# Video-Object-Detection/TSCD

Hardware: NVIDIA B200
Metric: clip-frames/sec of TSCD aggregation stage (higher is better)
Workload: dtype f16

## Files before the change

include/tscd_b200.h:

```cpp
#ifndef TSCD_B200_H_
#define TSCD_B200_H_

#include <stdint.h>

#ifdef __cplusplus
extern "C" {
#endif

#define TSCD_OK 0
#define TSCD_ERR_INVALID_ARG (-1)
#define TSCD_ERR_UNSUPPORTED (-2)
#define TSCD_ERR_CAPACITY (-3)
#define TSCD_ERR_CUDA (-4)

#define TSCD_F32 0
#define TSCD_F16 1
#define TSCD_BF16 2

#define TSCD_MAX_LEVELS 3

typedef struct {
    const void* ptr[TSCD_MAX_LEVELS];
    int64_t frame_stride[TSCD_MAX_LEVELS];
    int64_t anchor_stride[TSCD_MAX_LEVELS];
// ... 153 lines not shown
typedef struct {
    tscd_attn_layout lay;
    int32_t rows;
    const int32_t* m_dev;
    const void* x;
    int64_t ldx;
    const void* w;
    const int32_t* row_meta;
    const float* key_score;
    float scale;
    void *qn, *kn, *vn;
    void* vt;
    void* xori;
    int32_t ld_xori;
} tscd_qkv_project_args;
int tscd_qkv_project(const tscd_qkv_project_args* args, void* stream);

typedef struct {
    tscd_attn_layout lay;
    int32_t* row_frame;
    int32_t* row_meta;
    void* vt_cls;
    void* vt_reg;
} tscd_attn_rowmeta_args;
int tscd_attn_rowmeta(const tscd_attn_rowmeta_args* args, void* stream);

typedef struct {
    tscd_attn_layout lay;
    const void *qn_cls, *kn_cls, *qn_reg, *kn_reg;
    const void *vt_cls, *vt_reg;
    const int32_t* row_frame;
    int32_t need_reg;
    void* x_cls;
    void* x_reg;
    int32_t ld_x;
    float* stats;
    float max_logit;
} tscd_attn_pv_args;
int tscd_attn_pv(const tscd_attn_pv_args* args, void* stream);

typedef struct {
    tscd_attn_layout lay;
    const void *qn_cls, *kn_cls, *qn_reg, *kn_reg, *vn_cls, *vn_reg;
    const void* vt;
    const int32_t* row_frame;
    const float* stats;
    int32_t use_obj_mask;
    float sim_thresh;
    float conf_sim_thresh;
    void* out;
    int32_t ld_out;
    void* w_out;
    const void* w_in;
} tscd_attn_round2_args;
int tscd_attn_round2(const tscd_attn_round2_args* args, void* stream);

typedef struct {
    tscd_attn_layout lay;
    int32_t width;
    const void* x;
    int32_t ld_x;
    void* xt;
} tscd_transpose_args;
int tscd_transpose_clip(const tscd_transpose_args* args, void* stream);

typedef struct {
    int32_t B, F, L, D;
    int32_t bank_dtype;
    const int32_t* row_off;
    const int32_t* lrow_off;
    const void* bank_reg;
    const void* bank_edge;
    const float* time_emb;
    const float* se_w1;
    const float* se_w2;
    const float* emb_reg;
    const float* emb_cls;
    float* feat;
    float* edge;
    void* feat16;
    void* kin16;
    float* kin;
    float* norm_reg;
    float* norm_cls;
    int32_t emb_dtype;
} tscd_cafm_prep_args;
int tscd_cafm_prep(const tscd_cafm_prep_args* args, void* stream);

typedef struct {
    int32_t B, L, D, kmax;
    const int32_t* lrow_off;
    const int32_t* resume;
    const int32_t* st_n;
    const float* emb_reg; const float* emb_cls; const float* norm_reg; const float* norm_cls;
    const float* st_reg; const float* st_cls; const float* st_nreg; const float* st_ncls;
    float* cost;
    int32_t* ref_n;
    int32_t emb_dtype;
    const void* emb_reg16;
    const void* emb_cls16;
    int32_t emb16_dtype;
} tscd_cafm_cost_args;
int tscd_cafm_cost(const tscd_cafm_cost_args* args, void* stream);

typedef struct {
    int32_t num_frames, kmax;
// ... 246 lines not shown
```

tscd_b200/_lib.py:

```python
import ctypes as C
import os

from .build import LIB_PATH

TSCD_F32, TSCD_F16, TSCD_BF16 = 0, 1, 2
MAX_LEVELS = 3
_ERR = {-1: "invalid argument", -2: "unsupported configuration", -3: "capacity exceeded", -4: "CUDA error"}


class View(C.Structure):
    _fields_ = [("ptr", C.c_void_p * MAX_LEVELS), ("frame_stride", C.c_int64 * MAX_LEVELS),
                ("anchor_stride", C.c_int64 * MAX_LEVELS), ("chan_stride", C.c_int64 * MAX_LEVELS)]


class Anchors(C.Structure):
    _fields_ = [("num_levels", C.c_int32), ("level_h", C.c_int32 * MAX_LEVELS), ("level_w", C.c_int32 * MAX_LEVELS),
                ("level_stride", C.c_int32 * MAX_LEVELS), ("level_start", C.c_int32 * (MAX_LEVELS + 1))]


class SelectArgs(C.Structure):
    _fields_ = [("mode", C.c_int32), ("num_frames", C.c_int32), ("num_classes", C.c_int32), ("head_dtype", C.c_int32),
                ("apply_sigmoid", C.c_int32), ("apply_decode", C.c_int32), ("pre_k", C.c_int32),
                ("conf_thresh", C.c_float), ("minimal_limit", C.c_int32), ("maximal_limit", C.c_int32),
                ("cand_cap", C.c_int32), ("anchors", Anchors), ("reg", View), ("obj", View), ("cls", View),
# ... 23 lines not shown
                ("bank_dtype", C.c_int32), ("anchors", Anchors), ("reg", View), ("obj", View), ("cls", View),
                ("feat_cls", View), ("feat_reg", View), ("feat_edge", View),
                ("cand_idx", C.c_void_p), ("cand_count", C.c_void_p), ("keep", C.c_void_p), ("keep_count", C.c_void_p),
                ("sel_count", C.c_void_p), ("row_off", C.c_void_p), ("sel_idx", C.c_void_p), ("sel_rows", C.c_void_p),
                ("bank_cls", C.c_void_p), ("bank_reg", C.c_void_p), ("bank_edge", C.c_void_p),
                ("bank_score", C.c_void_p), ("bank_fg", C.c_void_p), ("bank_box", C.c_void_p)]


class LinearArgs(C.Structure):
    _fields_ = [("M", C.c_int32), ("N", C.c_int32), ("K", C.c_int32), ("dtype", C.c_int32),
                ("x", C.c_void_p), ("ldx", C.c_int64), ("w", C.c_void_p), ("ldw", C.c_int64),
                ("bias", C.c_void_p), ("m_dev", C.c_void_p), ("out16", C.c_void_p), ("ld16", C.c_int32),
                ("out32", C.c_void_p), ("ld32", C.c_int32)]


class AttnLayout(C.Structure):
    _fields_ = [("B", C.c_int32), ("F", C.c_int32), ("L", C.c_int32), ("self_attn", C.c_int32), ("dtype", C.c_int32),
                ("row_cap", C.c_int32), ("nk_pitch", C.c_int32), ("row_off", C.c_void_p), ("lrow_off", C.c_void_p)]


class AttnPrepArgs(C.Structure):
    _fields_ = [("lay", AttnLayout), ("scale", C.c_float), ("qkv_cls", C.c_void_p), ("qkv_reg", C.c_void_p),
                ("ld_qkv", C.c_int32), ("key_score", C.c_void_p),
                ("qn_cls", C.c_void_p), ("kn_cls", C.c_void_p), ("vn_cls", C.c_void_p),
                ("qn_reg", C.c_void_p), ("kn_reg", C.c_void_p), ("vn_reg", C.c_void_p),
                ("vt_cls", C.c_void_p), ("vt_reg", C.c_void_p), ("xori_cls", C.c_void_p), ("xori_reg", C.c_void_p),
                ("ld_xori", C.c_int32), ("row_frame", C.c_void_p)]


class QkvProjectArgs(C.Structure):
    _fields_ = [("lay", AttnLayout), ("rows", C.c_int32), ("m_dev", C.c_void_p), ("x", C.c_void_p), ("ldx", C.c_int64),
                ("w", C.c_void_p), ("row_meta", C.c_void_p), ("key_score", C.c_void_p), ("scale", C.c_float),
                ("qn", C.c_void_p), ("kn", C.c_void_p), ("vn", C.c_void_p), ("vt", C.c_void_p), ("xori", C.c_void_p),
                ("ld_xori", C.c_int32)]


class AttnRowmetaArgs(C.Structure):
    _fields_ = [("lay", AttnLayout), ("row_frame", C.c_void_p), ("row_meta", C.c_void_p), ("vt_cls", C.c_void_p),
                ("vt_reg", C.c_void_p)]


class AttnPvArgs(C.Structure):
    _fields_ = [("lay", AttnLayout), ("qn_cls", C.c_void_p), ("kn_cls", C.c_void_p), ("qn_reg", C.c_void_p),
                ("kn_reg", C.c_void_p), ("vt_cls", C.c_void_p), ("vt_reg", C.c_void_p), ("row_frame", C.c_void_p),
                ("need_reg", C.c_int32), ("x_cls", C.c_void_p), ("x_reg", C.c_void_p), ("ld_x", C.c_int32),
                ("stats", C.c_void_p), ("max_logit", C.c_float)]


class AttnRound2Args(C.Structure):
    _fields_ = [("lay", AttnLayout), ("qn_cls", C.c_void_p), ("kn_cls", C.c_void_p), ("qn_reg", C.c_void_p),
                ("kn_reg", C.c_void_p), ("vn_cls", C.c_void_p), ("vn_reg", C.c_void_p), ("vt", C.c_void_p),
                ("row_frame", C.c_void_p), ("stats", C.c_void_p), ("use_obj_mask", C.c_int32),
                ("sim_thresh", C.c_float), ("conf_sim_thresh", C.c_float), ("out", C.c_void_p), ("ld_out", C.c_int32),
                ("w_out", C.c_void_p), ("w_in", C.c_void_p)]


class TransposeArgs(C.Structure):
    _fields_ = [("lay", AttnLayout), ("width", C.c_int32), ("x", C.c_void_p), ("ld_x", C.c_int32), ("xt", C.c_void_p)]


def _fields(spec):
    m = {"i": C.c_int32, "f": C.c_float, "p": C.c_void_p}
    return [(x.split(":")[0], m[x.split(":")[1]]) for x in spec.split()]


class CafmPrepArgs(C.Structure):
    _fields_ = _fields("B:i F:i L:i D:i bank_dtype:i row_off:p lrow_off:p bank_reg:p bank_edge:p time_emb:p se_w1:p "
                       "se_w2:p emb_reg:p emb_cls:p feat:p edge:p feat16:p kin16:p kin:p norm_reg:p norm_cls:p emb_dtype:i")


class CafmChainArgs(C.Structure):
    _fields_ = _fields("B:i F:i L:i D:i kmax:i out_dtype:i row_off:p lrow_off:p resume:p feat:p edge:p kin:p kproj:p "
                       "vproj:p kproj16:p vproj16:p wq16:p bank_reg:p bank_edge:p time_emb:p emb_reg:p emb_cls:p norm_reg:p norm_cls:p wq_t:p se_w1:p se_w2:p ln_w:p "
                       "ln_b:p dec_w:p dec_b:p st_n:p st_out:p st_edge:p st_reg:p st_cls:p st_nreg:p st_ncls:p "
                       "st_time:p sc_qin:p sc_q:p sc_k:p ref_n:p lap_col:p lap_row:p out16:p out32:p perm:p status:p emb_dtype:i")


class CafmWideArgs(C.Structure):
    _fields_ = [("base", CafmChainArgs)] + _fields("qin16:p attn:p q_beg:p q_end:p kv_beg:p kv_end:p ctl:p perm_s:p prow_s:p ord_prev:p "
                                                   "n_prev:p last_l0:p")


class FrameFlashArgs(C.Structure):
    _fields_ = _fields("num_items:i heads:i head_dim:i dtype:i max_q:i q_beg:p q_end:p kv_beg:p kv_end:p q:p ldq:i k:p ldk:i v:p ldv:i "
                       "out:p ldo:i")


class EdgePatchesArgs(C.Structure):
    _fields_ = [("num_frames", C.c_int32), ("max_keep", C.c_int32), ("feat_dtype", C.c_int32), ("op_dtype", C.c_int32),
                ("anchors", Anchors), ("feat_reg", View), ("sel_idx", C.c_void_p), ("sel_count", C.c_void_p), ("row_off", C.c_void_p),
                ("seg_base", C.c_int32 * MAX_LEVELS), ("seg_cap", C.c_int32 * MAX_LEVELS), ("level_count", C.c_void_p),
                ("slot", C.c_void_p), ("patches", C.c_void_p), ("hf", C.c_void_p), ("status", C.c_void_p)]


class EdgeCombineArgs(C.Structure):
    _fields_ = _fields("rows_cap:i op_dtype:i total_rows:p slot:p content:p hf_out:p bank_edge:p")


class CafmCostArgs(C.Structure):
    _fields_ = _fields("B:i L:i D:i kmax:i lrow_off:p resume:p st_n:p emb_reg:p emb_cls:p norm_reg:p norm_cls:p "
                       "st_reg:p st_cls:p st_nreg:p st_ncls:p cost:p ref_n:p emb_dtype:i emb_reg16:p emb_cls16:p emb16_dtype:i")


class CafmLapArgs(C.Structure):
    _fields_ = _fields("num_frames:i kmax:i lrow_off:p ref_n:p cost:p lap_col:p lap_row:p")


# ... 149 lines not shown
```

tscd_b200/aggregate.py:

```python
from typing import Dict, Optional

import torch

import os

SINGLE_PASS_MAX_LOGIT = float(os.environ.get("TSCD_ATTN_MAX_LOGIT", "25.0"))

from . import ops

FUSED_QKV = True


class MCAWeights:

    def __init__(self, sd: Dict[str, torch.Tensor], prefix: str, dtype=torch.float16, device="cuda"):
        def w(name):
            return sd[prefix + name].detach().to(device=device, dtype=dtype).contiguous()

        def b(name):
            return sd[prefix + name].detach().to(device=device, dtype=torch.float32).contiguous()

        self.qkv_cls = torch.cat([w("mca.q_cls_local.weight"), w("mca.kv_cls.weight")], 0).contiguous()
        self.qkv_reg = torch.cat([w("mca.q_reg_local.weight"), w("mca.kv_reg.weight")], 0).contiguous()
        self.lin_w, self.lin_b = w("mca.linear.weight"), b("mca.linear.bias")
# ... 28 lines not shown
                                     xori_cls=tmp_c[:, 256:], xori_reg=tmp_r[:, 256:], tag=tag)
    else:
        qkv_c, _ = ops.linear(bank_cls, w.qkv_cls, m_dev=n_rows_dev)
        qkv_r, _ = ops.linear(bank_reg, w.qkv_reg, m_dev=n_rows_dev)
        bufs = ops.attn_prep(lay, qkv_c, qkv_r, bank_score, xori_cls=tmp_c[:, 256:], xori_reg=tmp_r[:, 256:])
    stats = torch.empty(lay.loc_cap, 16, dtype=torch.float32, device=dev)
    ops.attn_pv(lay, bufs, tmp_c[:, :256], tmp_r[:, :256], stats, need_reg=need_reg, tag=tag, max_logit=SINGLE_PASS_MAX_LOGIT)
    cat_c = torch.empty(lay.loc_cap, 768, dtype=dt, device=dev)
    ops.linear(tmp_c, w.lin_w, w.lin_b, m_dev=n_loc_dev, out16=cat_c[:, 256:], want16=False, tag=tag + ".mca_linear")
    w_keep = torch.empty(lay.loc_cap, lay.nk_pitch, dtype=dt, device=dev) if need_reg else None
    ops.attn_round2(lay, bufs, bufs["vt_cls"], stats, cat_c[:, :256], use_obj_mask=False, sim_thresh=sim_thresh,
                    conf_sim_thresh=conf_sim_thresh, w_out=w_keep, tag=tag + ".cls")
    trans_cls16, trans_cls32 = ops.linear(cat_c, w.out_w, w.out_b, m_dev=n_loc_dev, want16=cls_out[0], want32=cls_out[1],
                                          tag=tag + ".linear")
    trans_obj16 = trans_obj32 = None
    cat_r = None
    if need_reg:
        cat_r = torch.empty(lay.loc_cap, 768, dtype=dt, device=dev)
        ops.linear(tmp_r, w.linreg_w, w.linreg_b, m_dev=n_loc_dev, out16=cat_r[:, 256:], want16=False, tag=tag + ".mca_linear_reg")
        ops.attn_round2(lay, bufs, bufs["vt_reg"], stats, cat_r[:, :256], use_obj_mask=True, sim_thresh=sim_thresh,
                        conf_sim_thresh=conf_sim_thresh, w_in=w_keep, tag=tag + ".obj")
        trans_obj16, trans_obj32 = ops.linear(cat_r, w.obj_w, w.obj_b, m_dev=n_loc_dev, want16=obj_out[0], want32=obj_out[1],
                                              tag=tag + ".linear_obj")
    if debug is not None:
        debug.update(qkv_c=qkv_c, qkv_r=qkv_r, bufs=bufs, tmp_c=tmp_c, tmp_r=tmp_r, stats=stats, cat_c=cat_c, cat_r=cat_r)
    return (trans_cls16, trans_cls32), (trans_obj16, trans_obj32)


class MSAWeights:

    def __init__(self, sd: Dict[str, torch.Tensor], prefix: str, dtype=torch.float16, device="cuda"):
        w = lambda n: sd[prefix + n].detach().to(device=device, dtype=dtype).contiguous()
        b = lambda n: sd[prefix + n].detach().to(device=device, dtype=torch.float32).contiguous()
        self.qkv_cls, self.qkv_reg = w("msa.qkv_cls.weight"), w("msa.qkv_reg.weight")
        self.l1_w, self.l1_b = w("linear1.weight"), b("linear1.bias")
        self.l2_w, self.l2_b = w("linear2.weight"), b("linear2.bias")


def msa_forward(lay: ops.AttnLayoutT, w: MSAWeights, bank_cls, bank_reg, bank_score, n_rows_dev,
                sim_thresh=0.75, conf_sim_thresh=0.99):
    assert lay.self_attn and lay.L == lay.F
    dev, dt, cap = bank_cls.device, lay.dtype, lay.row_cap
    qkv_c, _ = ops.linear(bank_cls, w.qkv_cls, m_dev=n_rows_dev, tag="msa.qkv_cls")
    qkv_r, _ = ops.linear(bank_reg, w.qkv_reg, m_dev=n_rows_dev, tag="msa.qkv_reg")
    tmp_c = torch.empty(cap, 512, dtype=dt, device=dev)
    tmp_r = torch.empty(cap, 512, dtype=dt, device=dev)
    bufs = ops.attn_prep(lay, qkv_c, qkv_r, bank_score, xori_cls=tmp_c[:, 256:], xori_reg=tmp_r[:, 256:])
    stats = torch.empty(cap, 16, dtype=torch.float32, device=dev)
    ops.attn_pv(lay, bufs, tmp_c[:, :256], tmp_r[:, :256], stats, need_reg=False, tag="msa", max_logit=SINGLE_PASS_MAX_LOGIT)
    cat = torch.empty(cap, 1024, dtype=dt, device=dev)
    ops.linear(tmp_c, w.l1_w, w.l1_b, m_dev=n_rows_dev, out16=cat[:, 512:], want16=False, tag="msa.linear1")
    tct = torch.empty(lay.B * 512, lay.nk_pitch, dtype=dt, device=dev)
    ops.call("tscd_transpose_clip", ops.L.TransposeArgs, lay=lay.to_c(), width=512, x=cat[:, 512:], ld_x=cat.stride(0), xt=tct)
    for half in range(2):
        vt = tct.view(lay.B, 512, lay.nk_pitch)[:, half * 256:(half + 1) * 256]
        vt = vt.contiguous().view(lay.B * 256, lay.nk_pitch)
        ops.attn_round2(lay, bufs, vt, stats, cat[:, half * 256:(half + 1) * 256], use_obj_mask=False,
                        sim_thresh=sim_thresh, conf_sim_thresh=conf_sim_thresh, tag=f"msa.half{half}")
    return ops.linear(cat, w.l2_w, w.l2_b, m_dev=n_rows_dev, want16=True, want32=True, tag="msa.linear2")
```

tscd_b200/csrc/attn.cu:

```cuda
#include <cuda.h>

#include "common.cuh"
#include "tc.cuh"

namespace tscd {

int make_tmap_kmajor(CUtensorMap* m, const void* ptr, int is_bf16, int64_t rows, int64_t K, int64_t ld, int box_rows);

constexpr int kAttnThreads = 160;
constexpr float kLog2e = 1.4426950408889634f;

template <typename T>
__device__ __forceinline__ float2 ld2(const T* p);
template <> __device__ __forceinline__ float2 ld2<__half>(const __half* p) { return __half22float2(*reinterpret_cast<const __half2*>(p)); }
template <> __device__ __forceinline__ float2 ld2<__nv_bfloat16>(const __nv_bfloat16* p) {
    return __bfloat1622float2(*reinterpret_cast<const __nv_bfloat162*>(p));
}
template <typename T>
__device__ __forceinline__ void st2(T* p, float a, float b);
template <> __device__ __forceinline__ void st2<__half>(__half* p, float a, float b) { *reinterpret_cast<__half2*>(p) = __floats2half2_rn(a, b); }
template <> __device__ __forceinline__ void st2<__nv_bfloat16>(__nv_bfloat16* p, float a, float b) {
    *reinterpret_cast<__nv_bfloat162*>(p) = __floats2bfloat162_rn(a, b);
}

// ... 544 lines not shown
            softmax_bar_sync();
            lc = (bars.xch[0][row] + bars.xch[1][row]) + (bars.xch[2][row] + bars.xch[3][row]);
            softmax_bar_sync();
            bars.xch[quarter][row] = lr;
            softmax_bar_sync();
            lr = (bars.xch[0][row] + bars.xch[1][row]) + (bars.xch[2][row] + bars.xch[3][row]);
            softmax_bar_sync();
            lsum_c[h] = lc; lsum_r[h] = lr;
            PV_WAIT(&bars.o_full, h & 1, 352);
            tc_fence_after();
            const float ic = 0.5f / lc, ir = 0.5f / lr;
            for (int br = 0; br < (need_reg ? 2 : 1); ++br) {
                uint16_t* dst = reinterpret_cast<uint16_t*>(br == 0 ? a.x_cls : a.x_reg);
                const int c0 = quarter * 16;
                uint32_t oc[16], orr[16];
                tmem_ld_32x16(lane_base + (need_reg ? 256 + br * 64 : 256) + c0, oc);
                tmem_ld_32x16(lane_base + (need_reg ? 384 + br * 64 : 320) + c0, orr);
                tmem_ld_wait();
                if (q_ok) {
                    uint32_t pk[8];
#pragma unroll
                    for (int j = 0; j < 8; ++j)
                        pk[j] = pack2<BF16>(__uint_as_float(oc[2 * j]) * ic + __uint_as_float(orr[2 * j]) * ir,
                                            __uint_as_float(oc[2 * j + 1]) * ic + __uint_as_float(orr[2 * j + 1]) * ir);
                    uint4* o = reinterpret_cast<uint4*>(dst + (int64_t)(ci.lbase + q) * a.ld_x + h * 64 + c0);
#pragma unroll
                    for (int j = 0; j < 2; ++j) o[j] = make_uint4(pk[4 * j], pk[4 * j + 1], pk[4 * j + 2], pk[4 * j + 3]);
                }
            }
            tc_fence_before();
            __syncwarp();
            if (lane == 0) mbar_arrive(&bars.o_empty);
        }
        if (q_ok && quarter == 0) {
            float4* st = reinterpret_cast<float4*>(a.stats + (int64_t)(ci.lbase + q) * 16);
            st[0] = make_float4(mxc[0], mxc[1], mxc[2], mxc[3]);
            st[1] = make_float4(mxr[0], mxr[1], mxr[2], mxr[3]);
            st[2] = make_float4(lsum_c[0], lsum_c[1], lsum_c[2], lsum_c[3]);
            st[3] = make_float4(lsum_r[0], lsum_r[1], lsum_r[2], lsum_r[3]);
        }
    }
#ifdef TSCD_R2_PROF
    if (blockIdx.x == 0 && blockIdx.y == 0 && threadIdx.x == 0) atomicAdd(&g_pv_wait[63], (unsigned long long)(clock64() - tk0));
#endif
    tc_fence_before();
    __syncthreads();
    if (warp == 17) {
        tc_fence_after();
        tmem_dealloc<512>(tmem);
    }
}

struct R2Tmaps {
    CUtensorMap q128c, q128r, k64c, k64r, vn128c, vn128r, vn64c, vn64r, vt;
};

constexpr int kR2Threads = 640;
constexpr int kR2MaxSlots = 16;
constexpr int kR2SlotBytes = 8192;
constexpr int kR2SmemBytes = 229376;

struct R2Bars {
    uint64_t full[kR2MaxSlots], empty[kR2MaxSlots];
    uint64_t res_full;
    uint64_t r_full[2], r_empty[2];
    uint64_t s_full[2], s_empty[2];
    uint64_t w_full[2], w_empty[2];
    uint64_t u_full;
    uint32_t tmem_base;
    float xch[4][128];
};

static_assert(kR2SmemBytes + sizeof(R2Bars) <= 232448, "attn_round2: over the 227 KB shared-memory window");

struct R2Ring {
    int first, count;
    int pos;
    uint32_t ph;
    __device__ __forceinline__ R2Ring(int f, int c) : first(f), count(c), pos(f), ph(0) {}
    __device__ __forceinline__ int next(int n) {
        if (pos + n > first + count) pos = first;
        const int s = pos;
        pos += n;
        return s;
    }
    __device__ __forceinline__ uint32_t parity(int s) {
        const uint32_t p = (ph >> s) & 1u;
        ph ^= 1u << s;
        return p;
    }
};

template <class F>
__device__ __forceinline__ void r2_x_schedule(int KT, int atom0, int atom1, F&& f) {
    for (int x = atom0; x < atom1; ++x) f(1, 0, x);
    for (int kt = 0; kt < KT; ++kt) {
        if (kt >= 1) { f(2, kt - 1, 0); f(2, kt - 1, 1); }
        if (kt + 1 < KT)
            for (int x = atom0; x < atom1; ++x) f(1, kt + 1, x);
    }
    f(2, KT - 1, 0); f(2, KT - 1, 1);
}

template <bool BF16>
__global__ void __launch_bounds__(kR2Threads, 1) attn_round2_kernel(const __grid_constant__ R2Tmaps tm,
                                                                     const tscd_attn_round2_args a) {
    using namespace tc;
    const tscd_attn_layout& lay = a.lay;
    const int b = blockIdx.y;
    const ClipInfo ci = clip_info(lay, b, blockIdx.x);
    if (ci.q0 >= ci.n_loc) return;
#ifdef TSCD_R2_PROF
    const long long tk0 = clock64();
#endif

    extern __shared__ __align__(1024) unsigned char smem_raw[];
    unsigned char* smem = smem_raw;
    if ((smem_u32(smem) & 1023u) != 0) __trap();
    const bool use_obj = a.use_obj_mask != 0;
    const bool reuse = a.w_in != nullptr;
    const int n_atoms = use_obj ? 8 : 4;
    const int n_s = reuse ? 0 : 4, n_x = reuse ? 16 : 6;
    const int atom0 = reuse ? 4 : 0, atom1 = reuse ? 8 : n_atoms;
    unsigned char* sRes = smem;
    unsigned char* sRing = smem + (reuse ? 65536 : 131072);
    unsigned char* sW = sRing + (n_s + n_x) * kR2SlotBytes;
    R2Bars& bars = *reinterpret_cast<R2Bars*>(smem + kR2SmemBytes);

    const int warp = threadIdx.x >> 5, lane = threadIdx.x & 31;
    if (threadIdx.x == 512) {
        tma_prefetch_desc(&tm.q128c); tma_prefetch_desc(&tm.q128r); tma_prefetch_desc(&tm.k64c); tma_prefetch_desc(&tm.k64r);
        tma_prefetch_desc(&tm.vn128c); tma_prefetch_desc(&tm.vn128r); tma_prefetch_desc(&tm.vn64c); tma_prefetch_desc(&tm.vn64r);
        tma_prefetch_desc(&tm.vt);
        for (int i = 0; i < kR2MaxSlots; ++i) { mbar_init(&bars.full[i], 1); mbar_init(&bars.empty[i], 1); }
        mbar_init(&bars.res_full, 1);
        for (int i = 0; i < 2; ++i) {
            mbar_init(&bars.r_full[i], 1); mbar_init(&bars.r_empty[i], 16);
            mbar_init(&bars.s_full[i], 1); mbar_init(&bars.s_empty[i], 16);
            mbar_init(&bars.w_full[i], 16); mbar_init(&bars.w_empty[i], 1);
        }
        mbar_init(&bars.u_full, 1);
        fence_barrier_init();
    }
    if (warp == 17) tmem_alloc<512>(&bars.tmem_base);
    tc_fence_before();
    __syncthreads();
    tc_fence_after();
    const uint32_t tmem = bars.tmem_base;
    const int KT = (ci.n_clip + 63) / 64;
    if (warp == 16) {
        if (lane == 0) {
            if (reuse) {
                mbar_expect_tx(&bars.res_full, 4 * 16384);
                for (int at = 0; at < 4; ++at) tma_load_2d(sRes + at * 16384, &tm.vn128r, &bars.res_full, at * 64, ci.s0 + ci.q0);
            } else {
                mbar_expect_tx(&bars.res_full, 8 * 16384);
                for (int u = 0; u < 8; ++u)
                    tma_load_2d(sRes + u * 16384, (u & 1) == 0 ? &tm.q128c : &tm.q128r, &bars.res_full, (u >> 1) * 64, ci.s0 + ci.q0);
                R2Ring ring(0, n_s);
                for (int kt = 0; kt < KT; ++kt)
                    for (int u = 0; u < 8; ++u) {
                        const int sl = ring.next(1);
                        R2_WAIT(&bars.empty[sl], ring.parity(sl) ^ 1u, 400);
                        mbar_expect_tx(&bars.full[sl], 8192);
                        tma_load_2d(sRing + sl * kR2SlotBytes, (u & 1) == 0 ? &tm.k64c : &tm.k64r, &bars.full[sl], (u >> 1) * 64, ci.s0 + kt * 64);
                    }
            }
        }
    } else if (warp == 18) {
        if (lane == 0) {
            R2Ring ring(n_s, n_x);
            r2_x_schedule(KT, atom0, atom1, [&](int kind, int kt, int i) {
                const int n = kind == 2 ? 2 : (reuse ? 1 : 3);
                const int sl = ring.next(n);
                for (int j = 0; j < n; ++j) R2_WAIT(&bars.empty[sl + j], ring.parity(sl + j) ^ 1u, 401);
                uint64_t* fb = &bars.full[sl];
                unsigned char* d = sRing + sl * kR2SlotBytes;
                mbar_expect_tx(fb, n * 8192);
                if (kind == 1) {
                    const int br = i >> 2, at = i & 3;
                    if (reuse) {
                        tma_load_2d(d, &tm.vn64r, fb, at * 64, ci.s0 + kt * 64);
                    } else {
                        tma_load_2d(d, br == 0 ? &tm.vn128c : &tm.vn128r, fb, at * 64, ci.s0 + ci.q0);
                        tma_load_2d(d + 16384, br == 0 ? &tm.vn64c : &tm.vn64r, fb, at * 64, ci.s0 + kt * 64);
                    }
                } else {
                    tma_load_2d(d, &tm.vt, fb, kt * 64, b * 256 + i * 128);
                    tma_load_2d(d + 8192, &tm.vt, fb, kt * 64, b * 256 + i * 128 + 64);
                }
            });
        }
    } else if (warp == 17) {
        if (!reuse) {
            const uint32_t idesc64 = make_idesc_f16(BF16, 128, 64);
            R2Ring ring(0, n_s);
            R2_WAIT(&bars.res_full, 0, 414);
            tc_fence_after();
            uint32_t iu = 0;
            for (int kt = 0; kt < KT; ++kt)
                for (int u = 0; u < 8; ++u, ++iu) {
                    const int su = iu & 1;
                    R2_WAIT(&bars.s_empty[su], ((iu >> 1) & 1) ^ 1, 412);
                    const int sl = ring.next(1);
                    R2_WAIT(&bars.full[sl], ring.parity(sl), 410);
                    tc_fence_after();
                    const uint64_t dq = make_smem_desc_sw128(smem_u32(sRes + u * 16384));
                    const uint64_t dk = make_smem_desc_sw128(smem_u32(sRing + sl * kR2SlotBytes));
                    if (elect_one()) {
#pragma unroll
                        for (int k = 0; k < 4; ++k) umma_f16(tmem + 384 + su * 64, dq + 2 * k, dk + 2 * k, idesc64, k ? 1u : 0u);
                        umma_commit(&bars.empty[sl]);
                        umma_commit(&bars.s_full[su]);
                    }
                    __syncwarp();
                }
        }
    } else if (warp == 19) {
        {
            const uint32_t idesc64 = make_idesc_f16(BF16, 128, 64);
            const uint32_t idesc128 = make_idesc_f16(BF16, 128, 128);
            R2Ring ring(n_s, n_x);
            if (reuse) {
                R2_WAIT(&bars.res_full, 0, 414);
                tc_fence_after();
            }
            r2_x_schedule(KT, atom0, atom1, [&](int kind, int kt, int i) {
                const int n = kind == 2 ? 2 : (reuse ? 1 : 3);
                if (kind == 1) {
                    const int br = i >> 2, at = i & 3;
                    const int rb = reuse ? (kt & 1) : 0, use = reuse ? (kt >> 1) : kt;
                    if (i == atom0) {
                        R2_WAIT(&bars.r_empty[rb], (use & 1) ^ 1, 411);
                        tc_fence_after();
                    }
                    const int sl = ring.next(n);
                    R2_WAIT(&bars.full[sl], ring.parity(sl), 415);
                    tc_fence_after();
                    unsigned char* d = sRing + sl * kR2SlotBytes;
                    const uint64_t da = make_smem_desc_sw128(smem_u32(reuse ? sRes + at * 16384 : d));
                    const uint64_t db = make_smem_desc_sw128(smem_u32(reuse ? d : d + 16384));
                    const uint32_t col = tmem + 256 + (reuse ? rb : br) * 64;
                    if (elect_one()) {
#pragma unroll
                        for (int k = 0; k < 4; ++k) umma_f16(col, da + 2 * k, db + 2 * k, idesc64, (at | k) ? 1u : 0u);
                        for (int j = 0; j < n; ++j) umma_commit(&bars.empty[sl + j]);
                        if (i == atom1 - 1) umma_commit(&bars.r_full[rb]);
                    }
                    __syncwarp();
                } else {
                    const int wb = reuse ? (kt & 1) : 0, use = reuse ? (kt >> 1) : kt;
                    if (i == 0) {
                        R2_WAIT(&bars.w_full[wb], use & 1, 413);
                        tc_fence_after();
                    }
                    const int sl = ring.next(2);
                    R2_WAIT(&bars.full[sl], ring.parity(sl), 415);
                    tc_fence_after();
                    const uint64_t dw = make_smem_desc_sw128(smem_u32(sW + wb * 16384));
                    const uint64_t dv = make_smem_desc_sw128(smem_u32(sRing + sl * kR2SlotBytes));
                    if (elect_one()) {
#pragma unroll
                        for (int k = 0; k < 4; ++k) umma_f16(tmem + i * 128, dw + 2 * k, dv + 2 * k, idesc128, (kt | k) ? 1u : 0u);
                        umma_commit(&bars.empty[sl]);
                        umma_commit(&bars.empty[sl + 1]);
                        if (i == 1) umma_commit(&bars.w_empty[wb]);
                    }
                    __syncwarp();
                }
            });
            if (elect_one()) umma_commit(&bars.u_full);
            __syncwarp();
        }
    } else {
        constexpr int NC = 16;
        const int row = threadIdx.x & 127;
        const int quarter = (threadIdx.x >> 7) & 3;
        const int q = ci.q0 + row;
        const bool q_ok = q < ci.n_loc;
        const bool self_attn = lay.self_attn != 0;
        int lo = 0, hi = 0;
        if (q_ok && !self_attn) {
            const int qf = a.row_frame[ci.s0 + q];
            lo = lay.row_off[b * lay.F + qf] - ci.s0;
            hi = lay.row_off[b * lay.F + qf + 1] - ci.s0;
        }
        const int n_glob0 = self_attn ? 0 : ci.n_loc;
        const uint32_t lane_base = tmem + ((uint32_t)((warp & 3) * 32) << 16);
        float mcl[8], il[8];
#pragma unroll
        for (int u = 0; u < 8; ++u) { mcl[u] = 0.f; il[u] = 0.f; }
        if (q_ok && !reuse) {
            const float* st = a.stats + (int64_t)(ci.lbase + q) * 16;
#pragma unroll
            for (int h = 0; h < 4; ++h) {
                mcl[2 * h] = st[h] * kLog2e; mcl[2 * h + 1] = st[4 + h] * kLog2e;
                il[2 * h] = 0.5f / st[8 + h]; il[2 * h + 1] = 0.5f / st[12 + h];
            }
        }
        const int c0 = quarter * NC;
        auto range_bits = [](int k0, int k1, int base) -> uint32_t {
            const int x0 = min(max(k0 - base, 0), NC), x1 = min(max(k1 - base, 0), NC);
            return x1 > x0 ? (((1u << x1) - 1u) & ~((1u << x0) - 1u)) : 0u;
        };
        float den = 0.f;
        uint32_t iu = 0;
        for (int kt = 0; kt < KT; ++kt) {
            const int kbase = kt * 64;
            uint32_t bits = range_bits(n_glob0, ci.n_clip, kbase + c0) | range_bits(lo, min(hi, ci.n_clip), kbase + c0);
            const int rb = reuse ? (kt & 1) : 0, ruse = reuse ? (kt >> 1) : kt;
            R2_WAIT(&bars.r_full[rb], ruse & 1, 420);
            tc_fence_after();
            {
                uint32_t rc[NC], rr[NC];
                if (!reuse) tmem_ld_32x16(lane_base + 256 + c0, rc);
                if (use_obj) tmem_ld_32x16(lane_base + (reuse ? 256 + rb * 64 : 320) + c0, rr);
                tmem_ld_wait();
                uint32_t pass = 0;
#pragma unroll
                for (int j = 0; j < NC; ++j) {
                    bool ok = true;
                    if (!reuse) ok = __uint_as_float(rc[j]) * 0.25f > a.sim_thresh;
                    if (use_obj) ok = ok && (__uint_as_float(rr[j]) * 0.25f > a.conf_sim_thresh);
                    pass |= ok ? (1u << j) : 0u;
                }
                bits &= pass;
            }
            tc_fence_before();
            __syncwarp();
            if (lane == 0) mbar_arrive(&bars.r_empty[rb]);
            float w[NC];
            if (!reuse) {
                float as[NC];
#pragma unroll
                for (int j = 0; j < NC; ++j) as[j] = 0.f;
#pragma unroll
                for (int u = 0; u < 8; ++u, ++iu) {
                    const int su = iu & 1;
                    R2_WAIT(&bars.s_full[su], (iu >> 1) & 1, 421);
                    tc_fence_after();
                    uint32_t r[NC];
                    tmem_ld_32x16(lane_base + 384 + su * 64 + c0, r);
                    tmem_ld_wait();
                    tc_fence_before();
                    __syncwarp();
                    if (lane == 0) mbar_arrive(&bars.s_empty[su]);
                    const float m = mcl[u], sc = il[u];
#pragma unroll
                    for (int j = 0; j < NC; ++j) as[j] = fmaf(ex2_approx(fmaf(__uint_as_float(r[j]), kLog2e, -m)), sc, as[j]);
                }
#pragma unroll
                for (int j = 0; j < NC; ++j) w[j] = ((bits >> j) & 1u) ? ex2_approx(as[j] * (0.25f * kLog2e)) : 0.f;
            } else {
                const uint4* src = reinterpret_cast<const uint4*>(reinterpret_cast<const uint16_t*>(a.w_in) +
                                                                  (int64_t)(ci.lbase + min(q, ci.n_loc - 1)) * lay.nk_pitch + kbase + c0);
#pragma unroll
                for (int cc = 0; cc < NC / 8; ++cc) {
                    const uint4 raw = __ldg(src + cc);
                    const uint32_t wd[4] = {raw.x, raw.y, raw.z, raw.w};
#pragma unroll
                    for (int e = 0; e < 4; ++e) {
                        float lo16, hi16;
                        if (BF16) {
                            lo16 = __uint_as_float(wd[e] << 16); hi16 = __uint_as_float(wd[e] & 0xffff0000u);
                        } else {
                            const __half2 h2 = *reinterpret_cast<const __half2*>(&wd[e]);
                            lo16 = __low2float(h2); hi16 = __high2float(h2);
                        }
                        const int j = cc * 8 + e * 2;
                        w[j] = ((bits >> j) & 1u) ? lo16 : 0.f;
                        w[j + 1] = ((bits >> (j + 1)) & 1u) ? hi16 : 0.f;
                    }
                }
            }
            float d0 = 0.f, d1 = 0.f;
#pragma unroll
            for (int j = 0; j < NC; j += 2) { d0 += w[j]; d1 += w[j + 1]; }
            den += d0 + d1;
            const int wb = reuse ? (kt & 1) : 0;
            R2_WAIT(&bars.w_empty[wb], (ruse & 1) ^ 1, 422);
            unsigned char* sWb = sW + wb * 16384;
#pragma unroll
            for (int cc = 0; cc < NC / 8; ++cc) {
                const uint4 pk = make_uint4(pack2<BF16>(w[cc * 8], w[cc * 8 + 1]), pack2<BF16>(w[cc * 8 + 2], w[cc * 8 + 3]),
                                            pack2<BF16>(w[cc * 8 + 4], w[cc * 8 + 5]), pack2<BF16>(w[cc * 8 + 6], w[cc * 8 + 7]));
                *reinterpret_cast<uint4*>(sWb + sw128_off(row, (c0 >> 3) + cc)) = pk;
                if (a.w_out && q_ok)
                    *reinterpret_cast<uint4*>(reinterpret_cast<uint16_t*>(a.w_out) + (int64_t)(ci.lbase + q) * lay.nk_pitch + kbase + c0 + cc * 8) = pk;
            }
            fence_proxy_async();
            __syncwarp();
            if (lane == 0) mbar_arrive(&bars.w_full[wb]);
        }
        bars.xch[quarter][row] = den;
        asm volatile("bar.sync 1, 512;\n" ::: "memory");
        den = (bars.xch[0][row] + bars.xch[1][row]) + (bars.xch[2][row] + bars.xch[3][row]);
        R2_WAIT(&bars.u_full, 0, 423);
        tc_fence_after();
        const float inv = 1.f / den;
        uint16_t* dst = reinterpret_cast<uint16_t*>(a.out);
#pragma unroll 1
        for (int cb = quarter * 64; cb < quarter * 64 + 64; cb += 32) {
            uint32_t u[32];
            tmem_ld_32x32(lane_base + cb, u);
            tmem_ld_wait();
            if (q_ok) {
                uint32_t pk[16];
#pragma unroll
                for (int j = 0; j < 16; ++j) pk[j] = pack2<BF16>(__uint_as_float(u[2 * j]) * inv, __uint_as_float(u[2 * j + 1]) * inv);
                uint4* o = reinterpret_cast<uint4*>(dst + (int64_t)(ci.lbase + q) * a.ld_out + cb);
#pragma unroll
                for (int j = 0; j < 4; ++j) o[j] = make_uint4(pk[4 * j], pk[4 * j + 1], pk[4 * j + 2], pk[4 * j + 3]);
            }
        }
    }
#ifdef TSCD_R2_PROF
    if (blockIdx.x == 0 && blockIdx.y == 0 && threadIdx.x == 0) atomicAdd(&g_r2_wait[63], (unsigned long long)(clock64() - tk0));
#endif
    tc_fence_before();
    __syncthreads();
    if (warp == 17) {
        tc_fence_after();
        tmem_dealloc<512>(tmem);
    }
}

static bool layout_ok(const tscd_attn_layout& l) {
    return l.B > 0 && l.F > 0 && l.L > 0 && l.L <= l.F && l.row_cap > 0 && l.nk_pitch > 0 && (l.nk_pitch % 128) == 0 &&
           l.row_off && l.lrow_off && (l.dtype == TSCD_F16 || l.dtype == TSCD_BF16);
}

}

extern "C" int tscd_attn_prep(const tscd_attn_prep_args* a, void* stream) {
    using namespace tscd;
    if (!a || !layout_ok(a->lay)) return TSCD_ERR_INVALID_ARG;
    cudaStream_t st = reinterpret_cast<cudaStream_t>(stream);
    dim3 grid(a->lay.nk_pitch / 64, a->lay.B);
    const size_t smem = 2 * 64 * kPrepRowPitch * 2;
    if (a->lay.dtype == TSCD_F16) {
        if (cudaFuncSetAttribute(attn_prep_kernel<__half>, cudaFuncAttributeMaxDynamicSharedMemorySize, (int)smem) != cudaSuccess) return TSCD_ERR_CUDA;
        attn_prep_kernel<__half><<<grid, kPrepThreads, smem, st>>>(*a);
    } else {
        if (cudaFuncSetAttribute(attn_prep_kernel<__nv_bfloat16>, cudaFuncAttributeMaxDynamicSharedMemorySize, (int)smem) != cudaSuccess) return TSCD_ERR_CUDA;
        attn_prep_kernel<__nv_bfloat16><<<grid, kPrepThreads, smem, st>>>(*a);
    }
    TSCD_CUDA_CHECK_LAUNCH();
    return TSCD_OK;
}

extern "C" int tscd_transpose_clip(const tscd_transpose_args* a, void* stream) {
    using namespace tscd;
    if (!a || !layout_ok(a->lay) || a->width <= 0 || (a->width % 64) != 0) return TSCD_ERR_INVALID_ARG;
    dim3 grid(a->lay.nk_pitch / 64, a->width / 64, a->lay.B);
    cudaStream_t st = reinterpret_cast<cudaStream_t>(stream);
    if (a->lay.dtype == TSCD_F16) transpose_clip_kernel<__half><<<grid, 256, 0, st>>>(*a);
    else transpose_clip_kernel<__nv_bfloat16><<<grid, 256, 0, st>>>(*a);
    TSCD_CUDA_CHECK_LAUNCH();
    return TSCD_OK;
}

extern "C" int tscd_attn_pv(const tscd_attn_pv_args* a, void* stream) {
    using namespace tscd;
    if (!a || !layout_ok(a->lay)) return TSCD_ERR_INVALID_ARG;
    const tscd_attn_layout& l = a->lay;
    const int bf = l.dtype == TSCD_BF16;
    PvTmaps tm;
    int rc = 0;
    rc |= make_tmap_kmajor(&tm.qc, a->qn_cls, bf, l.row_cap, 256, 256, 128);
    rc |= make_tmap_kmajor(&tm.kc, a->kn_cls, bf, l.row_cap, 256, 256, 128);
    rc |= make_tmap_kmajor(&tm.qr, a->qn_reg, bf, l.row_cap, 256, 256, 128);
    rc |= make_tmap_kmajor(&tm.kr, a->kn_reg, bf, l.row_cap, 256, 256, 128);
    rc |= make_tmap_kmajor(&tm.k64c, a->kn_cls, bf, l.row_cap, 256, 256, 64);
    rc |= make_tmap_kmajor(&tm.k64r, a->kn_reg, bf, l.row_cap, 256, 256, 64);
    rc |= make_tmap_kmajor(&tm.vtc, a->vt_cls, bf, (int64_t)l.B * 256, l.nk_pitch, l.nk_pitch, 64);
    rc |= make_tmap_kmajor(&tm.vtr, a->vt_reg, bf, (int64_t)l.B * 256, l.nk_pitch, l.nk_pitch, 64);
    if (rc) return TSCD_ERR_CUDA;
    const size_t smem = 65536 + kPvStages * 32768 + 65536 + sizeof(PvBars);
    dim3 grid((l.nk_pitch + 127) / 128, l.B);
    cudaStream_t st = reinterpret_cast<cudaStream_t>(stream);
    if (bf) {
        if (cudaFuncSetAttribute(attn_pv_kernel<true>, cudaFuncAttributeMaxDynamicSharedMemorySize, (int)smem) != cudaSuccess) return TSCD_ERR_CUDA;
        attn_pv_kernel<true><<<grid, kPvThreads, smem, st>>>(tm, *a);
    } else {
        if (cudaFuncSetAttribute(attn_pv_kernel<false>, cudaFuncAttributeMaxDynamicSharedMemorySize, (int)smem) != cudaSuccess) return TSCD_ERR_CUDA;
        attn_pv_kernel<false><<<grid, kPvThreads, smem, st>>>(tm, *a);
    }
    TSCD_CUDA_CHECK_LAUNCH();
    return TSCD_OK;
}

extern "C" int tscd_attn_round2(const tscd_attn_round2_args* a, void* stream) {
    using namespace tscd;
    if (!a || !layout_ok(a->lay)) return TSCD_ERR_INVALID_ARG;
    if (a->w_in && !a->use_obj_mask) return TSCD_ERR_INVALID_ARG;
    const tscd_attn_layout& l = a->lay;
    const int bf = l.dtype == TSCD_BF16;
    R2Tmaps tm;
    int rc = 0;
    rc |= make_tmap_kmajor(&tm.q128c, a->qn_cls, bf, l.row_cap, 256, 256, 128);
    rc |= make_tmap_kmajor(&tm.q128r, a->qn_reg, bf, l.row_cap, 256, 256, 128);
    rc |= make_tmap_kmajor(&tm.k64c, a->kn_cls, bf, l.row_cap, 256, 256, 64);
    rc |= make_tmap_kmajor(&tm.k64r, a->kn_reg, bf, l.row_cap, 256, 256, 64);
    rc |= make_tmap_kmajor(&tm.vn128c, a->vn_cls, bf, l.row_cap, 256, 256, 128);
    rc |= make_tmap_kmajor(&tm.vn128r, a->vn_reg, bf, l.row_cap, 256, 256, 128);
    rc |= make_tmap_kmajor(&tm.vn64c, a->vn_cls, bf, l.row_cap, 256, 256, 64);
    rc |= make_tmap_kmajor(&tm.vn64r, a->vn_reg, bf, l.row_cap, 256, 256, 64);
    rc |= make_tmap_kmajor(&tm.vt, a->vt, bf, (int64_t)l.B * 256, l.nk_pitch, l.nk_pitch, 64);
    if (rc) return TSCD_ERR_CUDA;
    const size_t smem = kR2SmemBytes + sizeof(R2Bars);
    dim3 grid((l.nk_pitch + 127) / 128, l.B);
    cudaStream_t st = reinterpret_cast<cudaStream_t>(stream);
    if (bf) {
        if (cudaFuncSetAttribute(attn_round2_kernel<true>, cudaFuncAttributeMaxDynamicSharedMemorySize, (int)smem) != cudaSuccess) return TSCD_ERR_CUDA;
        attn_round2_kernel<true><<<grid, kR2Threads, smem, st>>>(tm, *a);
    } else {
        if (cudaFuncSetAttribute(attn_round2_kernel<false>, cudaFuncAttributeMaxDynamicSharedMemorySize, (int)smem) != cudaSuccess) return TSCD_ERR_CUDA;
        attn_round2_kernel<false><<<grid, kR2Threads, smem, st>>>(tm, *a);
    }
    TSCD_CUDA_CHECK_LAUNCH();
    return TSCD_OK;
}

#ifdef TSCD_R2_PROF
extern "C" int tscd_debug_r2_waits(unsigned long long* out, int reset) {
    if (reset) {
        unsigned long long z[64] = {};
        return cudaMemcpyToSymbol(tscd::g_r2_wait, z, sizeof(z)) == cudaSuccess && cudaMemcpyToSymbol(tscd::g_pv_wait, z, sizeof(z)) == cudaSuccess ? 0 : -1;
    }
    return cudaMemcpyFromSymbol(out, tscd::g_r2_wait, sizeof(unsigned long long) * 64) == cudaSuccess &&
                   cudaMemcpyFromSymbol(out + 64, tscd::g_pv_wait, sizeof(unsigned long long) * 64) == cudaSuccess ? 0 : -1;
}
#endif

extern "C" int tscd_attn_rowmeta(const tscd_attn_rowmeta_args* a, void* stream) {
    using namespace tscd;
    if (!a || !layout_ok(a->lay) || !a->row_frame || !a->row_meta || !a->vt_cls || a->lay.B > 32767 || a->lay.nk_pitch > 65536) return TSCD_ERR_INVALID_ARG;
    dim3 grid(a->lay.nk_pitch / 64, a->lay.B);
    cudaStream_t st = reinterpret_cast<cudaStream_t>(stream);
    if (a->lay.dtype == TSCD_F16) attn_rowmeta_kernel<__half><<<grid, 64, 0, st>>>(*a);
    else attn_rowmeta_kernel<__nv_bfloat16><<<grid, 64, 0, st>>>(*a);
    TSCD_CUDA_CHECK_LAUNCH();
    return TSCD_OK;
}
```

tscd_b200/ops.py:

```python
import ctypes as C
from dataclasses import dataclass
from typing import List, Optional, Sequence

import torch

from . import _lib as L

_DT = {torch.float32: L.TSCD_F32, torch.float16: L.TSCD_F16, torch.bfloat16: L.TSCD_BF16}


def _stream():
    return C.c_void_p(torch.cuda.current_stream().cuda_stream)


def _p(t: Optional[torch.Tensor]):
    return C.c_void_p(0 if t is None else t.data_ptr())


@dataclass
class AnchorSpec:
    hw: Sequence[Sequence[int]]
    strides: Sequence[int] = (8, 16, 32)

    @property
# ... 384 lines not shown
    assert qkv_cls.stride(1) == 1 and qkv_cls.stride(0) == qkv_reg.stride(0)
    a.qkv_cls, a.qkv_reg, a.ld_qkv, a.key_score = _p(qkv_cls), _p(qkv_reg), qkv_cls.stride(0), _p(key_score)
    for n in ("qn_cls", "kn_cls", "vn_cls", "qn_reg", "kn_reg", "vn_reg", "vt_cls", "vt_reg", "row_frame"):
        setattr(a, n, _p(bufs[n]))
    a.xori_cls, a.xori_reg = _p(xori_cls), _p(xori_reg)
    a.ld_xori = 0 if xori_cls is None else xori_cls.stride(0)
    with L.timed("tscd_attn_prep"):
        L.check(L.lib().tscd_attn_prep(C.byref(a), _stream()), "tscd_attn_prep")
    return bufs


def qkv_project_fused(lay: AttnLayoutT, bank_cls, bank_reg, w_cls, w_reg, key_score, n_rows_dev, xori_cls=None, xori_reg=None,
                      scale=25.0, tag=None):
    dev, dt = bank_cls.device, lay.dtype
    bufs = {}
    for n in ("qn_cls", "kn_cls", "vn_cls", "qn_reg", "kn_reg", "vn_reg"):
        bufs[n] = torch.empty(lay.row_cap, 256, dtype=dt, device=dev)
    for n in ("vt_cls", "vt_reg"):
        bufs[n] = torch.empty(lay.B * 256, lay.nk_pitch, dtype=dt, device=dev)
    bufs["row_frame"] = torch.empty(lay.row_cap, dtype=torch.int32, device=dev)
    bufs["row_meta"] = torch.empty(lay.row_cap, dtype=torch.int32, device=dev)
    call("tscd_attn_rowmeta", L.AttnRowmetaArgs, lay=lay.to_c(), row_frame=bufs["row_frame"], row_meta=bufs["row_meta"],
         vt_cls=bufs["vt_cls"], vt_reg=bufs["vt_reg"])
    for br, bank, w, ks, xo in (("cls", bank_cls, w_cls, key_score, xori_cls), ("reg", bank_reg, w_reg, None, xori_reg)):
        assert bank.shape[0] >= lay.row_cap and bank.stride(1) == 1 and w.shape == (768, 256) and w.is_contiguous()
        call("tscd_qkv_project", L.QkvProjectArgs, tag=None if tag is None else f"{tag}.{br}", lay=lay.to_c(), rows=lay.row_cap, m_dev=n_rows_dev, x=bank, ldx=bank.stride(0),
             w=w, row_meta=bufs["row_meta"], key_score=ks, scale=scale, qn=bufs["qn_" + br], kn=bufs["kn_" + br],
             vn=bufs["vn_" + br], vt=bufs["vt_" + br], xori=xo, ld_xori=0 if xo is None else xo.stride(0))
    return bufs


def attn_pv(lay: AttnLayoutT, bufs, x_cls, x_reg, stats, need_reg=True, tag=None, max_logit: float = 0.0):
    a = L.AttnPvArgs()
    a.max_logit = max_logit
    a.lay = lay.to_c()
    for n in ("qn_cls", "kn_cls", "qn_reg", "kn_reg", "vt_cls", "vt_reg", "row_frame"):
        setattr(a, n, _p(bufs[n]))
    a.need_reg = int(need_reg)
    a.x_cls, a.x_reg, a.ld_x, a.stats = _p(x_cls), _p(x_reg), x_cls.stride(0), _p(stats)
    with L.timed("tscd_attn_pv", tag):
        L.check(L.lib().tscd_attn_pv(C.byref(a), _stream()), "tscd_attn_pv")


def attn_round2(lay: AttnLayoutT, bufs, vt, stats, out, use_obj_mask, sim_thresh=0.75, conf_sim_thresh=0.99, w_out=None, w_in=None,
                tag=None):
    a = L.AttnRound2Args()
    a.lay = lay.to_c()
    for n in ("qn_cls", "kn_cls", "qn_reg", "kn_reg", "vn_cls", "vn_reg", "row_frame"):
        setattr(a, n, _p(bufs[n]))
    a.vt, a.stats, a.use_obj_mask = _p(vt), _p(stats), int(use_obj_mask)
    a.sim_thresh, a.conf_sim_thresh = sim_thresh, conf_sim_thresh
    a.out, a.ld_out = _p(out), out.stride(0)
    a.w_out, a.w_in = _p(w_out), _p(w_in)
    for t in (w_out, w_in):
        assert t is None or (t.dtype == lay.dtype and t.stride(0) == lay.nk_pitch and t.stride(1) == 1)
    with L.timed("tscd_attn_round2", tag):
        L.check(L.lib().tscd_attn_round2(C.byref(a), _stream()), "tscd_attn_round2")


def call(name: str, struct_cls, tag=None, **kw):
    a = struct_cls()
    for k, v in kw.items():
        if isinstance(v, C.Structure):
            pass
        elif isinstance(v, torch.Tensor) or v is None:
            v = _p(v)
        elif isinstance(v, torch.dtype):
            v = _DT[v]
        setattr(a, k, v)
    missing = {f[0] for f in struct_cls._fields_} - set(kw)
    assert not missing, f"{name}: missing {missing}"
    with L.timed(name, tag):
        L.check(getattr(L.lib(), name)(C.byref(a), _stream()), name)
```

Baseline: 1.528 million.

## Reuse round-2 attention weights across MSA halves via TMA-loaded smem buffer

The MSA round-2 attention runs twice, once per 256-wide half of V. The first half now writes its normalized attention weights to a buffer, and the second half reads them back instead of recomputing logits and softmax. The reuse path now loads those weights into shared memory with a TMA tensor map on double-buffered barriers, replacing per-thread global loads, and skips the residual/similarity wait when no object mask is used. The cost is an extra weight write and buffer allocation, plus more complex barrier logic with hang or race risk.

```diff
diff --git a/include/tscd_b200.h b/include/tscd_b200.h
--- a/include/tscd_b200.h
+++ b/include/tscd_b200.h
@@ -229,6 +229,7 @@
     int32_t ld_out;
     void* w_out;
     const void* w_in;
+    int32_t w_rows;
 } tscd_attn_round2_args;
 int tscd_attn_round2(const tscd_attn_round2_args* args, void* stream);
 
diff --git a/tscd_b200/_lib.py b/tscd_b200/_lib.py
--- a/tscd_b200/_lib.py
+++ b/tscd_b200/_lib.py
@@ -99,7 +99,7 @@
                 ("kn_reg", C.c_void_p), ("vn_cls", C.c_void_p), ("vn_reg", C.c_void_p), ("vt", C.c_void_p),
                 ("row_frame", C.c_void_p), ("stats", C.c_void_p), ("use_obj_mask", C.c_int32),
                 ("sim_thresh", C.c_float), ("conf_sim_thresh", C.c_float), ("out", C.c_void_p), ("ld_out", C.c_int32),
-                ("w_out", C.c_void_p), ("w_in", C.c_void_p)]
+                ("w_out", C.c_void_p), ("w_in", C.c_void_p), ("w_rows", C.c_int32)]
 
 
 class TransposeArgs(C.Structure):
diff --git a/tscd_b200/aggregate.py b/tscd_b200/aggregate.py
--- a/tscd_b200/aggregate.py
+++ b/tscd_b200/aggregate.py
@@ -104,9 +104,11 @@
     ops.linear(tmp_c, w.l1_w, w.l1_b, m_dev=n_rows_dev, out16=cat[:, 512:], want16=False, tag="msa.linear1")
     tct = torch.empty(lay.B * 512, lay.nk_pitch, dtype=dt, device=dev)
     ops.call("tscd_transpose_clip", ops.L.TransposeArgs, lay=lay.to_c(), width=512, x=cat[:, 512:], ld_x=cat.stride(0), xt=tct)
+    w_keep = torch.empty(cap, lay.nk_pitch, dtype=dt, device=dev)
     for half in range(2):
         vt = tct.view(lay.B, 512, lay.nk_pitch)[:, half * 256:(half + 1) * 256]
         vt = vt.contiguous().view(lay.B * 256, lay.nk_pitch)
         ops.attn_round2(lay, bufs, vt, stats, cat[:, half * 256:(half + 1) * 256], use_obj_mask=False,
-                        sim_thresh=sim_thresh, conf_sim_thresh=conf_sim_thresh, tag=f"msa.half{half}")
+                        sim_thresh=sim_thresh, conf_sim_thresh=conf_sim_thresh, w_out=None if half else w_keep,
+                        w_in=w_keep if half else None, tag=f"msa.half{half}")
     return ops.linear(cat, w.l2_w, w.l2_b, m_dev=n_rows_dev, want16=True, want32=True, tag="msa.linear2")
diff --git a/tscd_b200/csrc/attn.cu b/tscd_b200/csrc/attn.cu
--- a/tscd_b200/csrc/attn.cu
+++ b/tscd_b200/csrc/attn.cu
@@ -620,7 +620,7 @@
 }
 
 struct R2Tmaps {
-    CUtensorMap q128c, q128r, k64c, k64r, vn128c, vn128r, vn64c, vn64r, vt;
+    CUtensorMap q128c, q128r, k64c, k64r, vn128c, vn128r, vn64c, vn64r, vt, win;
 };
 
 constexpr int kR2Threads = 640;
@@ -634,6 +634,7 @@
     uint64_t r_full[2], r_empty[2];
     uint64_t s_full[2], s_empty[2];
     uint64_t w_full[2], w_empty[2];
+    uint64_t win_full[2];
     uint64_t u_full;
     uint32_t tmem_base;
     float xch[4][128];
@@ -687,9 +688,10 @@
     if ((smem_u32(smem) & 1023u) != 0) __trap();
     const bool use_obj = a.use_obj_mask != 0;
     const bool reuse = a.w_in != nullptr;
+    const bool need_r = !reuse || use_obj;
     const int n_atoms = use_obj ? 8 : 4;
     const int n_s = reuse ? 0 : 4, n_x = reuse ? 16 : 6;
-    const int atom0 = reuse ? 4 : 0, atom1 = reuse ? 8 : n_atoms;
+    const int atom0 = reuse ? 4 : 0, atom1 = reuse ? (use_obj ? 8 : 4) : n_atoms;
     unsigned char* sRes = smem;
     unsigned char* sRing = smem + (reuse ? 65536 : 131072);
     unsigned char* sW = sRing + (n_s + n_x) * kR2SlotBytes;
@@ -700,12 +702,14 @@
         tma_prefetch_desc(&tm.q128c); tma_prefetch_desc(&tm.q128r); tma_prefetch_desc(&tm.k64c); tma_prefetch_desc(&tm.k64r);
         tma_prefetch_desc(&tm.vn128c); tma_prefetch_desc(&tm.vn128r); tma_prefetch_desc(&tm.vn64c); tma_prefetch_desc(&tm.vn64r);
         tma_prefetch_desc(&tm.vt);
+        if (reuse) tma_prefetch_desc(&tm.win);
         for (int i = 0; i < kR2MaxSlots; ++i) { mbar_init(&bars.full[i], 1); mbar_init(&bars.empty[i], 1); }
         mbar_init(&bars.res_full, 1);
         for (int i = 0; i < 2; ++i) {
             mbar_init(&bars.r_full[i], 1); mbar_init(&bars.r_empty[i], 16);
             mbar_init(&bars.s_full[i], 1); mbar_init(&bars.s_empty[i], 16);
             mbar_init(&bars.w_full[i], 16); mbar_init(&bars.w_empty[i], 1);
+            mbar_init(&bars.win_full[i], 1);
         }
         mbar_init(&bars.u_full, 1);
         fence_barrier_init();
@@ -719,8 +723,16 @@
     if (warp == 16) {
         if (lane == 0) {
             if (reuse) {
-                mbar_expect_tx(&bars.res_full, 4 * 16384);
-                for (int at = 0; at < 4; ++at) tma_load_2d(sRes + at * 16384, &tm.vn128r, &bars.res_full, at * 64, ci.s0 + ci.q0);
+                if (use_obj) {
+                    mbar_expect_tx(&bars.res_full, 4 * 16384);
+                    for (int at = 0; at < 4; ++at) tma_load_2d(sRes + at * 16384, &tm.vn128r, &bars.res_full, at * 64, ci.s0 + ci.q0);
+                }
+                for (int kt = 0; kt < KT; ++kt) {
+                    const int wb = kt & 1;
+                    R2_WAIT(&bars.w_empty[wb], ((kt >> 1) & 1) ^ 1, 402);
+                    mbar_expect_tx(&bars.win_full[wb], 16384);
+                    tma_load_2d(sW + wb * 16384, &tm.win, &bars.win_full[wb], kt * 64, ci.lbase + ci.q0);
+                }
             } else {
                 mbar_expect_tx(&bars.res_full, 8 * 16384);
                 for (int u = 0; u < 8; ++u)
@@ -789,7 +801,7 @@
             const uint32_t idesc64 = make_idesc_f16(BF16, 128, 64);
             const uint32_t idesc128 = make_idesc_f16(BF16, 128, 128);
             R2Ring ring(n_s, n_x);
-            if (reuse) {
+            if (reuse && use_obj) {
                 R2_WAIT(&bars.res_full, 0, 414);
                 tc_fence_after();
             }
@@ -877,9 +889,9 @@
             const int kbase = kt * 64;
             uint32_t bits = range_bits(n_glob0, ci.n_clip, kbase + c0) | range_bits(lo, min(hi, ci.n_clip), kbase + c0);
             const int rb = reuse ? (kt & 1) : 0, ruse = reuse ? (kt >> 1) : kt;
-            R2_WAIT(&bars.r_full[rb], ruse & 1, 420);
-            tc_fence_after();
-            {
+            if (need_r) {
+                R2_WAIT(&bars.r_full[rb], ruse & 1, 420);
+                tc_fence_after();
                 uint32_t rc[NC], rr[NC];
                 if (!reuse) tmem_ld_32x16(lane_base + 256 + c0, rc);
                 if (use_obj) tmem_ld_32x16(lane_base + (reuse ? 256 + rb * 64 : 320) + c0, rr);
@@ -893,10 +905,12 @@
                     pass |= ok ? (1u << j) : 0u;
                 }
                 bits &= pass;
-            }
-            tc_fence_before();
-            __syncwarp();
-            if (lane == 0) mbar_arrive(&bars.r_empty[rb]);
+                tc_fence_before();
+                __syncwarp();
+                if (lane == 0) mbar_arrive(&bars.r_empty[rb]);
+            }
+            const int wb = reuse ? (kt & 1) : 0;
+            unsigned char* sWb = sW + wb * 16384;
             float w[NC];
             if (!reuse) {
                 float as[NC];
@@ -920,41 +934,40 @@
 #pragma unroll
                 for (int j = 0; j < NC; ++j) w[j] = ((bits >> j) & 1u) ? ex2_approx(as[j] * (0.25f * kLog2e)) : 0.f;
             } else {
-                const uint4* src = reinterpret_cast<const uint4*>(reinterpret_cast<const uint16_t*>(a.w_in) +
-                                                                  (int64_t)(ci.lbase + min(q, ci.n_loc - 1)) * lay.nk_pitch + kbase + c0);
+                R2_WAIT(&bars.win_full[wb], (kt >> 1) & 1, 424);
 #pragma unroll
                 for (int cc = 0; cc < NC / 8; ++cc) {
-                    const uint4 raw = __ldg(src + cc);
-                    const uint32_t wd[4] = {raw.x, raw.y, raw.z, raw.w};
+                    uint4* p = reinterpret_cast<uint4*>(sWb + sw128_off(row, (c0 >> 3) + cc));
+                    const uint4 raw = *p;
+                    uint32_t wd[4] = {raw.x, raw.y, raw.z, raw.w};
 #pragma unroll
                     for (int e = 0; e < 4; ++e) {
-                        float lo16, hi16;
+                        const int j = cc * 8 + e * 2;
+                        wd[e] &= (((bits >> j) & 1u) ? 0x0000ffffu : 0u) | (((bits >> (j + 1)) & 1u) ? 0xffff0000u : 0u);
                         if (BF16) {
-                            lo16 = __uint_as_float(wd[e] << 16); hi16 = __uint_as_float(wd[e] & 0xffff0000u);
+                            w[j] = __uint_as_float(wd[e] << 16); w[j + 1] = __uint_as_float(wd[e] & 0xffff0000u);
                         } else {
                             const __half2 h2 = *reinterpret_cast<const __half2*>(&wd[e]);
-                            lo16 = __low2float(h2); hi16 = __high2float(h2);
+                            w[j] = __low2float(h2); w[j + 1] = __high2float(h2);
                         }
-                        const int j = cc * 8 + e * 2;
-                        w[j] = ((bits >> j) & 1u) ? lo16 : 0.f;
-                        w[j + 1] = ((bits >> (j + 1)) & 1u) ? hi16 : 0.f;
-                    }
+                    }
+                    if (use_obj) *p = make_uint4(wd[0], wd[1], wd[2], wd[3]);
                 }
             }
             float d0 = 0.f, d1 = 0.f;
 #pragma unroll
             for (int j = 0; j < NC; j += 2) { d0 += w[j]; d1 += w[j + 1]; }
             den += d0 + d1;
-            const int wb = reuse ? (kt & 1) : 0;
-            R2_WAIT(&bars.w_empty[wb], (ruse & 1) ^ 1, 422);
-            unsigned char* sWb = sW + wb * 16384;
-#pragma unroll
-            for (int cc = 0; cc < NC / 8; ++cc) {
-                const uint4 pk = make_uint4(pack2<BF16>(w[cc * 8], w[cc * 8 + 1]), pack2<BF16>(w[cc * 8 + 2], w[cc * 8 + 3]),
-                                            pack2<BF16>(w[cc * 8 + 4], w[cc * 8 + 5]), pack2<BF16>(w[cc * 8 + 6], w[cc * 8 + 7]));
-                *reinterpret_cast<uint4*>(sWb + sw128_off(row, (c0 >> 3) + cc)) = pk;
-                if (a.w_out && q_ok)
-                    *reinterpret_cast<uint4*>(reinterpret_cast<uint16_t*>(a.w_out) + (int64_t)(ci.lbase + q) * lay.nk_pitch + kbase + c0 + cc * 8) = pk;
+            if (!reuse) {
+                R2_WAIT(&bars.w_empty[wb], (ruse & 1) ^ 1, 422);
+#pragma unroll
+                for (int cc = 0; cc < NC / 8; ++cc) {
+                    const uint4 pk = make_uint4(pack2<BF16>(w[cc * 8], w[cc * 8 + 1]), pack2<BF16>(w[cc * 8 + 2], w[cc * 8 + 3]),
+                                                pack2<BF16>(w[cc * 8 + 4], w[cc * 8 + 5]), pack2<BF16>(w[cc * 8 + 6], w[cc * 8 + 7]));
+                    *reinterpret_cast<uint4*>(sWb + sw128_off(row, (c0 >> 3) + cc)) = pk;
+                    if (a.w_out && q_ok)
+                        *reinterpret_cast<uint4*>(reinterpret_cast<uint16_t*>(a.w_out) + (int64_t)(ci.lbase + q) * lay.nk_pitch + kbase + c0 + cc * 8) = pk;
+                }
             }
             fence_proxy_async();
             __syncwarp();
@@ -1061,7 +1074,7 @@
 extern "C" int tscd_attn_round2(const tscd_attn_round2_args* a, void* stream) {
     using namespace tscd;
     if (!a || !layout_ok(a->lay)) return TSCD_ERR_INVALID_ARG;
-    if (a->w_in && !a->use_obj_mask) return TSCD_ERR_INVALID_ARG;
+    if (a->w_in && (a->w_out || a->w_rows <= 0)) return TSCD_ERR_INVALID_ARG;
     const tscd_attn_layout& l = a->lay;
     const int bf = l.dtype == TSCD_BF16;
     R2Tmaps tm;
@@ -1075,6 +1088,8 @@
     rc |= make_tmap_kmajor(&tm.vn64c, a->vn_cls, bf, l.row_cap, 256, 256, 64);
     rc |= make_tmap_kmajor(&tm.vn64r, a->vn_reg, bf, l.row_cap, 256, 256, 64);
     rc |= make_tmap_kmajor(&tm.vt, a->vt, bf, (int64_t)l.B * 256, l.nk_pitch, l.nk_pitch, 64);
+    if (a->w_in) rc |= make_tmap_kmajor(&tm.win, a->w_in, bf, a->w_rows, l.nk_pitch, l.nk_pitch, 128);
+    else memset(&tm.win, 0, sizeof(tm.win));
     if (rc) return TSCD_ERR_CUDA;
     const size_t smem = kR2SmemBytes + sizeof(R2Bars);
     dim3 grid((l.nk_pitch + 127) / 128, l.B);
diff --git a/tscd_b200/ops.py b/tscd_b200/ops.py
--- a/tscd_b200/ops.py
+++ b/tscd_b200/ops.py
@@ -460,6 +460,7 @@
     a.sim_thresh, a.conf_sim_thresh = sim_thresh, conf_sim_thresh
     a.out, a.ld_out = _p(out), out.stride(0)
     a.w_out, a.w_in = _p(w_out), _p(w_in)
+    a.w_rows = w_in.shape[0] if w_in is not None else 0
     for t in (w_out, w_in):
         assert t is None or (t.dtype == lay.dtype and t.stride(0) == lay.nk_pitch and t.stride(1) == 1)
     with L.timed("tscd_attn_round2", tag):
```

Measured after the change: 1.539 million, median of 6. About the same (+0.8%).
